# Roestlab/diffusion-deconvolution-dia-msms-data

Hardware: AMD Instinct MI355X
Metric: MS2 windows/s (train step: zero_grad + train_step + backward + clip 10 + AdamW) (higher is better)
Workload: dtype f32; 1 GPU; BASELINE configs[1]: default UNet1d (dim 4, mults 1,2,2,3,3,4,4; 128,847 params), synthetic MS2+MS1 windows 400 RT x 64 m/z, batch 32 per GPU, fp32; global_batch=32, parallelism=dp1

## Files before the change

### diffusion-deconvolution-dia-msms-data_amd/csrc/dq_mfma.h

```cpp
#pragma once
#include <hip/hip_runtime.h>

namespace dq {

typedef float f32x16 __attribute__((ext_vector_type(16)));

__device__ __forceinline__ f32x16 mfma_f32(float a, float b, f32x16 c) { return __builtin_amdgcn_mfma_f32_32x32x2f32(a, b, c, 0, 0, 0); }
__device__ __forceinline__ constexpr int rmap(int r, int half) { return (r & 3) + 8 * (r >> 2) + 4 * half; }
__host__ __device__ __forceinline__ constexpr int la_nj(int C) { return C == 4 ? 2 : (C == 12 ? 6 : (C <= 8 ? 4 : 8)); }
__device__ __forceinline__ constexpr int la_chan(int C, int j, int half) {
  return C == 4 ? 2 * half + j : (C == 12 ? 6 * half + j : rmap(j, half));
}
__host__ __device__ __forceinline__ constexpr int sm_chan(int C, int i, int half) { return C == 12 ? i + 6 * half : (i & 3) + 8 * (i >> 2) + 4 * half; }
__device__ __forceinline__ float swap_half(float v) { return __shfl_xor(v, 32, 64); }

__device__ __forceinline__ f32x16 xty(const f32x16& x, const f32x16& y, f32x16 acc) {
#pragma unroll
  for (int r = 0; r < 16; ++r) acc = mfma_f32(x[r], y[r], acc);
  return acc;
}

__device__ __forceinline__ f32x16 transpose_tile(f32x16 a, float* tile, int col, int half) {
  __builtin_amdgcn_fence(__ATOMIC_ACQ_REL, "wavefront");
  __builtin_amdgcn_wave_barrier();
#pragma unroll
  for (int r = 0; r < 16; ++r) tile[rmap(r, half) * 33 + col] = a[r];
  __builtin_amdgcn_fence(__ATOMIC_ACQ_REL, "wavefront");
  __builtin_amdgcn_wave_barrier();
  f32x16 o;
#pragma unroll
  for (int r = 0; r < 16; ++r) o[r] = tile[col * 33 + rmap(r, half)];
  return o;
}

template <int N>
__device__ __forceinline__ f32x16 mask_same_row(f32x16 a, int col, int half) {
  const int cr = col / N;
#pragma unroll
  for (int r = 0; r < 16; ++r) {
    const int rr = half ? rmap(r, 1) / N : rmap(r, 0) / N;
    a[r] = rr == cr ? a[r] : 0.f;
  }
  return a;
}

}
```

### diffusion-deconvolution-dia-msms-data_amd/csrc/k_attn.hip

```cpp
#include "dq_common.h"
#include "dq_kernels.h"
#include "dq_mfma.h"
#include <cstdlib>

namespace dq {


constexpr float ATT_SCALE = 0.17677669529663687f;
constexpr float LOG2E = 1.4426950408889634f;

__global__ void __launch_bounds__(256) k_rope(float* __restrict__ t0, int64_t bs0, float* __restrict__ t1, int64_t bs1, const float* __restrict__ freqs,
                                              int RT, float sign, int64_t total) {
  float* __restrict__ t = blockIdx.y ? t1 : t0;
  const int64_t batch_stride = blockIdx.y ? bs1 : bs0;
  const int64_t i = blockIdx.x * (int64_t)blockDim.x + threadIdx.x;
  if (i >= total) return;
  const int pos = (int)(i % RT);
  const int pr = (int)((i / RT) % 8);
  const int64_t bh = i / ((int64_t)RT * 8);
  const int64_t b = bh >> 2, h = bh & 3;
  const float ang = (float)pos * freqs[pr];
  float sn, cs;
  sincosf(ang, &sn, &cs);
  sn *= sign;
  float* pa = t + b * batch_stride + (h * 32 + 2 * pr) * RT + pos;
  const float xa = pa[0], xb = pa[RT];
  pa[0] = xa * cs - xb * sn;
  pa[RT] = xb * cs + xa * sn;
}

int launch_rope(float* qk, const float* freqs, int B, int64_t batch_stride, int RT, float sign, hipStream_t s) {
  const int64_t total = (int64_t)B * 4 * 8 * RT;
  if (total == 0) return 0;
  hipLaunchKernelGGL(k_rope, dim3(cdiv(total, 256)), dim3(256), 0, s, qk, batch_stride, (float*)nullptr, (int64_t)0, freqs, RT, sign, total);
  DQ_LAUNCH_CHECK();
  return 0;
}
int launch_rope2(float* q, int64_t q_bs, float* k, int64_t k_bs, const float* freqs, int B, int RT, float sign, hipStream_t s) {
  const int64_t total = (int64_t)B * 4 * 8 * RT;
  if (total == 0) return 0;
  hipLaunchKernelGGL(k_rope, dim3(cdiv(total, 256), 2), dim3(256), 0, s, q, q_bs, k, k_bs, freqs, RT, sign, total);
  DQ_LAUNCH_CHECK();
  return 0;
}

template <bool FAST = true>
__device__ __forceinline__ f32x16 tile_ch_rows(const float* __restrict__ src, int RT, int p0, int col, int half, float mul) {
  f32x16 t;
  if (FAST && p0 + 32 <= RT) {
    const unsigned voff = (unsigned)(p0 + col + 4 * half * RT) * 4u;
#pragma unroll
    for (int r = 0; r < 16; ++r) {
      const float v = *reinterpret_cast<const float*>(reinterpret_cast<const char*>(src + (size_t)((r & 3) + 8 * (r >> 2)) * RT) + voff);
      t[r] = mul == 1.f ? v : v * mul;
    }
    return t;
  }
  const int p = p0 + col;
  const bool ok = p < RT;
  const float* s0 = src + (ok ? p : RT - 1);
  const float m = ok ? mul : 0.f;
#pragma unroll
  for (int r = 0; r < 16; ++r) t[r] = s0[(int64_t)rmap(r, half) * RT] * m;
  return t;
}
__device__ __forceinline__ f32x16 tile_pos_rows(const float* __restrict__ src, int RT, int p0, int col, int half, float mul) {
  f32x16 t;
  const float* row = src + (int64_t)col * RT;
  if ((RT & 3) == 0 && p0 + 32 <= RT) {
#pragma unroll
    for (int q4 = 0; q4 < 4; ++q4) {
      const float4 v = *reinterpret_cast<const float4*>(row + p0 + 8 * q4 + 4 * half);
      if (mul == 1.f) { t[4 * q4 + 0] = v.x; t[4 * q4 + 1] = v.y; t[4 * q4 + 2] = v.z; t[4 * q4 + 3] = v.w; }
      else { t[4 * q4 + 0] = v.x * mul; t[4 * q4 + 1] = v.y * mul; t[4 * q4 + 2] = v.z * mul; t[4 * q4 + 3] = v.w * mul; }
    }
  } else {
#pragma unroll
    for (int r = 0; r < 16; ++r) {
      const int p = p0 + rmap(r, half);
      t[r] = row[p < RT ? p : RT - 1] * (p < RT ? mul : 0.f);
    }
  }
  return t;
}
__device__ __forceinline__ f32x16 rows_scalar(const float* __restrict__ v, int RT, int p0, int half, float fill) {
  f32x16 t;
#pragma unroll
  for (int r = 0; r < 16; ++r) {
    const int p = p0 + rmap(r, half);
    const float x = v[p < RT ? p : RT - 1];
    t[r] = p < RT ? x : fill;
  }
  return t;
}

__global__ void __launch_bounds__(64) k_attn_fwd(const float* __restrict__ q, int64_t q_bs, const float* __restrict__ k, int64_t k_bs,
                                                 const float* __restrict__ v, int64_t v_bs, float* __restrict__ o,
                                                 float* __restrict__ lse, int RT) {
  const int lane = threadIdx.x & 63, col = lane & 31, half = lane >> 5;
  const int bh = blockIdx.y, b = bh >> 2, h = bh & 3;
  const int i0 = blockIdx.x * 32, i = i0 + col;
  const float* qb = q + b * q_bs + (int64_t)h * 32 * RT;
  const float* kb = k + b * k_bs + (int64_t)h * 32 * RT;
  const float* vb = v + b * v_bs + (int64_t)h * 32 * RT;
  const f32x16 Qt = tile_ch_rows<false>(qb, RT, i0, col, half, ATT_SCALE);
  f32x16 Oa = {0};
  float m = -INFINITY, l = 0.f;
  const int jlast = (RT - 1) / 32 * 32;
  auto kblk = [&](int j) { return min(j, jlast); };
  f32x16 Kn = tile_ch_rows<false>(kb, RT, kblk(0), col, half, 1.f);
  f32x16 Vn = tile_pos_rows(vb, RT, kblk(0), col, half, 1.f);
  for (int j0 = 0; j0 < RT; j0 += 32) {
    const f32x16 Kt = Kn, Vx = Vn;
    Kn = tile_ch_rows<false>(kb, RT, kblk(j0 + 32), col, half, 1.f);
    Vn = tile_pos_rows(vb, RT, kblk(j0 + 32), col, half, 1.f);
    f32x16 St = xty(Kt, Qt, f32x16{0});
    float mx = -INFINITY;
#pragma unroll
    for (int r = 0; r < 16; ++r) {
      if (j0 + rmap(r, half) >= RT) St[r] = -INFINITY;
      mx = fmaxf(mx, St[r]);
    }
    mx = fmaxf(mx, swap_half(mx));
    const float mn = fmaxf(m, mx);
    const float al = __builtin_amdgcn_exp2f((m - mn) * LOG2E);
    float ls = 0.f;
#pragma unroll
    for (int r = 0; r < 16; ++r) {
      St[r] = __builtin_amdgcn_exp2f((St[r] - mn) * LOG2E);
      ls += St[r];
    }
    ls += swap_half(ls);
    l = fmaf(l, al, ls);
    m = mn;
#pragma unroll
    for (int r = 0; r < 16; ++r) Oa[r] *= al;
    Oa = xty(Vx, St, Oa);
  }
  if (i < RT) {
    const float rl = 1.0f / l;
    float* ob = o + (int64_t)b * 128 * RT + (int64_t)h * 32 * RT;
#pragma unroll
    for (int r = 0; r < 16; ++r) ob[(int64_t)rmap(r, half) * RT + i] = Oa[r] * rl;
    if (lse && half == 0) lse[(int64_t)bh * RT + i] = m + __logf(l);
  }
}

int launch_attn_fwd(const float* q, int64_t q_bs, const float* k, int64_t k_bs, const float* v, int64_t v_bs, float* o, float* lse,
                    int B, int RT, hipStream_t s) {
  if (B == 0 || RT == 0) return 0;
  hipLaunchKernelGGL(k_attn_fwd, dim3(cdiv(RT, 32), B * 4), dim3(64), 0, s, q, q_bs, k, k_bs, v, v_bs, o, lse, RT);
  DQ_LAUNCH_CHECK();
  return 0;
}

__global__ void __launch_bounds__(64) k_attn_bwd_q(const float* __restrict__ q, int64_t q_bs, const float* __restrict__ k,
                                                   int64_t k_bs, const float* __restrict__ v, int64_t v_bs,
                                                   const float* __restrict__ o, const float* __restrict__ d_o,
                                                   const float* __restrict__ lse, float* __restrict__ delta,
                                                   float* __restrict__ dq, int64_t dq_bs, int RT) {
  const int lane = threadIdx.x & 63, col = lane & 31, half = lane >> 5;
  const int bh = blockIdx.y, b = bh >> 2, h = bh & 3;
  const int i0 = blockIdx.x * 32, i = i0 + col;
  const float* qb = q + b * q_bs + (int64_t)h * 32 * RT;
  const float* kb = k + b * k_bs + (int64_t)h * 32 * RT;
  const float* vb = v + b * v_bs + (int64_t)h * 32 * RT;
  const float* ob = o + (int64_t)b * 128 * RT + (int64_t)h * 32 * RT;
  const float* dob = d_o + (int64_t)b * 128 * RT + (int64_t)h * 32 * RT;
  const int jlast = (RT - 1) / 32 * 32;
  auto kblk = [&](int j) { return min(j, jlast); };
  f32x16 Kn = tile_ch_rows(kb, RT, kblk(0), col, half, 1.f);
  f32x16 Vn = tile_ch_rows(vb, RT, kblk(0), col, half, 1.f);
  f32x16 Xn = tile_pos_rows(kb, RT, kblk(0), col, half, 1.f);
  const f32x16 Qt = tile_ch_rows(qb, RT, i0, col, half, ATT_SCALE);
  const f32x16 dOt = tile_ch_rows(dob, RT, i0, col, half, 1.f);
  float dl = 0.f;
  {
    const f32x16 Ot = tile_ch_rows(ob, RT, i0, col, half, 1.f);
#pragma unroll
    for (int r = 0; r < 16; ++r) dl = fmaf(dOt[r], Ot[r], dl);
    dl += swap_half(dl);
  }
  const float ls = i < RT ? lse[(int64_t)bh * RT + i] : INFINITY;
  f32x16 dQa = {0};
  for (int j0 = 0; j0 < RT; j0 += 32) {
    const f32x16 Kt = Kn, Vt = Vn, Kx = Xn;
    Kn = tile_ch_rows(kb, RT, kblk(j0 + 32), col, half, 1.f);
    Vn = tile_ch_rows(vb, RT, kblk(j0 + 32), col, half, 1.f);
    Xn = tile_pos_rows(kb, RT, kblk(j0 + 32), col, half, 1.f);
    f32x16 St = xty(Kt, Qt, f32x16{0});
    const f32x16 dPt = xty(Vt, dOt, f32x16{0});
#pragma unroll
    for (int r = 0; r < 16; ++r) {
      const float p = (j0 + rmap(r, half) < RT) ? __builtin_amdgcn_exp2f((St[r] - ls) * LOG2E) : 0.f;
      St[r] = p * (dPt[r] - dl);
    }
    dQa = xty(Kx, St, dQa);
  }
  if (i < RT) {
    float* dqb = dq + b * dq_bs + (int64_t)h * 32 * RT;
#pragma unroll
    for (int r = 0; r < 16; ++r) dqb[(int64_t)rmap(r, half) * RT + i] = dQa[r] * ATT_SCALE;
    if (half == 0) delta[(int64_t)bh * RT + i] = dl;
  }
}

__global__ void __launch_bounds__(256, 2) k_attn_bwd_kv(const float* __restrict__ q, int64_t q_bs, const float* __restrict__ k,
                                                     int64_t k_bs, const float* __restrict__ v, int64_t v_bs,
                                                     const float* __restrict__ d_o, const float* __restrict__ lse,
                                                     const float* __restrict__ delta, float* __restrict__ dk, int64_t dk_bs,
                                                     float* __restrict__ dv, int64_t dv_bs, int RT) {
  const int lane = threadIdx.x & 63, col = lane & 31, half = lane >> 5;
  const int wv = __builtin_amdgcn_readfirstlane(threadIdx.x >> 6);
  const int bh = blockIdx.y, b = bh >> 2, h = bh & 3;
  const int j0 = blockIdx.x * 32, j = j0 + col;
  const float* qb = q + b * q_bs + (int64_t)h * 32 * RT;
  const float* kb = k + b * k_bs + (int64_t)h * 32 * RT;
  const float* vb = v + b * v_bs + (int64_t)h * 32 * RT;
  const float* dob = d_o + (int64_t)b * 128 * RT + (int64_t)h * 32 * RT;
  const float* lsb = lse + (int64_t)bh * RT;
  const float* dlb = delta + (int64_t)bh * RT;
  const int ilast = (RT - 1) / 32 * 32;
  f32x16 Qn = tile_ch_rows(qb, RT, min(wv * 32, ilast), col, half, ATT_SCALE), dOn = tile_ch_rows(dob, RT, min(wv * 32, ilast), col, half, 1.f);
  const f32x16 Kt = tile_ch_rows(kb, RT, j0, col, half, 1.f);
  const f32x16 Vt = tile_ch_rows(vb, RT, j0, col, half, 1.f);
  f32x16 dKa = {0}, dVa = {0};
  __shared__ float ttiles[4][32 * 33];
  __shared__ float acc_lds[3][2][16][64];
  float* ttile = ttiles[wv];
  for (int i0 = wv * 32; i0 < RT; i0 += 128) {
    const f32x16 Qt = Qn, dOt = dOn;
    const f32x16 lsr = rows_scalar(lsb, RT, i0, half, INFINITY);
    const f32x16 dlr = rows_scalar(dlb, RT, i0, half, 0.f);
    Qn = tile_ch_rows(qb, RT, min(i0 + 128, ilast), col, half, ATT_SCALE);
    dOn = tile_ch_rows(dob, RT, min(i0 + 128, ilast), col, half, 1.f);
    f32x16 S = xty(Qt, Kt, f32x16{0});
#pragma unroll
    for (int r = 0; r < 16; ++r) S[r] = __builtin_amdgcn_exp2f((S[r] - lsr[r]) * LOG2E);
    {
      const f32x16 dOx = transpose_tile(dOt, ttile, col, half);
      dVa = xty(dOx, S, dVa);
    }
    __builtin_amdgcn_sched_barrier(0);
    f32x16 dP = xty(dOt, Vt, f32x16{0});
#pragma unroll
    for (int r = 0; r < 16; ++r) dP[r] = S[r] * (dP[r] - dlr[r]);
    {
      const f32x16 Qx = transpose_tile(Qt, ttile, col, half);
      dKa = xty(Qx, dP, dKa);
    }
  }
  if (wv > 0) {
#pragma unroll
    for (int r = 0; r < 16; ++r) { acc_lds[wv - 1][0][r][lane] = dKa[r]; acc_lds[wv - 1][1][r][lane] = dVa[r]; }
  }
  __syncthreads();
  if (wv == 0 && j < RT) {
    float* dkb = dk + b * dk_bs + (int64_t)h * 32 * RT;
    float* dvb = dv + b * dv_bs + (int64_t)h * 32 * RT;
#pragma unroll
    for (int r = 0; r < 16; ++r) {
      const float sk = ((dKa[r] + acc_lds[0][0][r][lane]) + acc_lds[1][0][r][lane]) + acc_lds[2][0][r][lane];
      const float sv = ((dVa[r] + acc_lds[0][1][r][lane]) + acc_lds[1][1][r][lane]) + acc_lds[2][1][r][lane];
      dkb[(int64_t)rmap(r, half) * RT + j] = sk;
      dvb[(int64_t)rmap(r, half) * RT + j] = sv;
    }
  }
}

int launch_attn_bwd(const float* q, int64_t q_bs, const float* k, int64_t k_bs, const float* v, int64_t v_bs, const float* o,
                    const float* d_o, const float* lse, float* delta, float* dq, int64_t dq_bs, float* dk, int64_t dk_bs, float* dv,
                    int64_t dv_bs, int B, int RT, hipStream_t s) {
  if (B == 0 || RT == 0) return 0;
  dim3 grid(cdiv(RT, 32), B * 4);
  hipLaunchKernelGGL(k_attn_bwd_q, grid, dim3(64), 0, s, q, q_bs, k, k_bs, v, v_bs, o, d_o, lse, delta, dq, dq_bs, RT);
  DQ_LAUNCH_CHECK();
  hipLaunchKernelGGL(k_attn_bwd_kv, grid, dim3(256), 0, s, q, q_bs, k, k_bs, v, v_bs, d_o, lse, delta, dk, dk_bs, dv, dv_bs, RT);
  DQ_LAUNCH_CHECK();
  return 0;
}

}
```

### diffusion-deconvolution-dia-msms-data_amd/csrc/k_linattn.hip

```cpp
#include "dq_common.h"
#include "dq_kernels.h"
#include "dq_mfma.h"
#include "dq_probe.h"
#include <algorithm>
#include <cstdlib>
#include <string>

namespace dq {

typedef float f32x4 __attribute__((ext_vector_type(4)));
__device__ __forceinline__ f32x16 mfma32(float a, float b, f32x16 c) { return __builtin_amdgcn_mfma_f32_32x32x2f32(a, b, c, 0, 0, 0); }
__device__ __forceinline__ f32x4 mfma4f(float a, float b, f32x4 c) { return __builtin_amdgcn_mfma_f32_4x4x1f32(a, b, c, 0, 0, 0); }
__device__ __forceinline__ constexpr int rowmap(int r, int half) { return (r & 3) + 8 * (r >> 2) + 4 * half; }
__device__ __forceinline__ float swap32(float v) { return swap_half(v); }
__device__ __forceinline__ void wave_fence() {
  __builtin_amdgcn_fence(__ATOMIC_ACQ_REL, "wavefront");
  __builtin_amdgcn_wave_barrier();
}

typedef __bf16 bf16x8 __attribute__((ext_vector_type(8)));
typedef unsigned int u32x4 __attribute__((ext_vector_type(4)));
__host__ __device__ __forceinline__ constexpr int la_nu(int C) { return (3 * (C / 2) + 3) / 4; }
__device__ __forceinline__ bf16x8 as_bf16x8(u32x4 v) { union { u32x4 u; bf16x8 b; } c; c.u = v; return c.b; }
__device__ __forceinline__ void la_split_x(float v, unsigned& d0, unsigned& d1, unsigned& d2) {
  const unsigned vb = __float_as_uint(v);
  const float r = v - __uint_as_float(vb & 0xffff0000u);
  const unsigned rb = __float_as_uint(r);
  const float l = r - __uint_as_float(rb & 0xffff0000u);
  d0 = __builtin_amdgcn_perm(vb, vb, 0x07060706u);
  d1 = __builtin_amdgcn_perm(rb, rb, 0x07060706u);
  d2 = __builtin_amdgcn_perm(__float_as_uint(l), vb, 0x07060302u);
}
__device__ __forceinline__ unsigned la_bf16_image_dword(const float* __restrict__ w_qkv, int C, int o, int half, int u, int e) {
  const int dw = 4 * u + e, j = dw / 3, t = dw % 3;
  if (j >= C / 2) return 0u;
  const float w = w_qkv[o * C + la_chan(C, j, half)] * 1.4426950408889634f;
  const unsigned hb = __float_as_uint(w) & 0xffff0000u;
  const float r = w - __uint_as_float(hb);
  const unsigned mb = __float_as_uint(r) & 0xffff0000u;
  const unsigned lb = __float_as_uint(r - __uint_as_float(mb));
  return t < 2 ? ((hb >> 16) | mb) : ((lb >> 16) | hb);
}

template <int C, int N, bool BF>
__global__ void __launch_bounds__(256) k_linattn_fwd(LinAttn a) {
  static_assert(!BF || (C <= 8 && N > 1), "the bf16 operand image of 12 / 16 channels does not fit the static LDS next to the other images");
  constexpr int NU = la_nu(C);
  constexpr int NB = N >= 32 ? N / 32 : 1;
  constexpr int RW = N >= 32 ? 1 : 32 / N;
  constexpr int NJ = la_nj(C);
  constexpr int SEG = N >= 32 ? 16 : (N >= 8 ? N / 2 : N);
  constexpr bool PARTNER = N >= 8;
  constexpr int CG = C / 4;
  constexpr int NP = NB * 32;
  constexpr bool SEGM = N == 8 || N == 16;
  static_assert(NB <= 2, "rows longer than 64 take the two-pass path (k_la_long.hip)");
  static_assert(C % 4 == 0, "channel count must be a multiple of 4");

  __shared__ __attribute__((aligned(16))) float w2_lds[4 * C * C];
  __shared__ __attribute__((aligned(16))) float xs_lds[4][C * NP];
  constexpr int MS_ROW = C * 32 + 8;
  __shared__ __attribute__((aligned(16))) float ms_lds[4][(SEGM ? RW : 1) * MS_ROW];
  constexpr bool QUAD = N > 1 && N < 32 && !SEGM;
  __shared__ float tiles[QUAD ? 4 : 1][QUAD ? 32 * 33 : 1];
  float* tile = tiles[QUAD ? (threadIdx.x >> 6) : 0];
  DQ_PSTAMP(300000 + C * 100 + N, 0);
#ifdef DQ_KPROBE
  if ((threadIdx.x & 63) == 0 && threadIdx.x > 0 && dq_kprobe_want == 300000 + C * 100 + N)
    dq_kprobe_buf[((blockIdx.y * gridDim.x + blockIdx.x) & 4095) * 16 + 5 + (threadIdx.x >> 6)] = clock64();
#endif
  const int lane = threadIdx.x & 63, col = lane & 31, half = lane >> 5, wv = threadIdx.x >> 6;
  const int rl = N >= 32 ? 0 : col / N;
  const int unit0 = blockIdx.x * 4 + wv, ustride = gridDim.x * 4;
  float Xn[NB][NJ], gpre_r[NJ], gout_r[NJ], bout_r[NJ];
  auto request_unit = [&](int unit) __attribute__((always_inline)) {
    const int rq = unit * RW + rl;
    const int rc = rq < a.rows ? rq : a.rows - 1;
#pragma unroll
    for (int blk = 0; blk < NB; ++blk) {
      const int pos = N >= 32 ? blk * 32 + col : col % N;
#pragma unroll
      for (int j = 0; j < NJ; ++j) {
        const int c = la_chan(C, j, half);
        Xn[blk][j] = a.x[((int64_t)rc * C + (c < C ? c : 0)) * N + pos];
      }
    }
  };
  auto request_x = [&]() __attribute__((always_inline)) {
    request_unit(unit0);
#pragma unroll
    for (int j = 0; j < NJ; ++j) {
      const int c = la_chan(C, j, half);
      gpre_r[j] = a.g_pre[c < C ? c : 0];
      gout_r[j] = a.g_out[c < C ? c : 0];
      bout_r[j] = a.b_out[c < C ? c : 0];
    }
  };
  float bflag = 0.f;
  constexpr int WQ = BF ? 2 * 4 * NU * 64 * 4 : 2 * 4 * NJ * 2 * 32;
  __shared__ __attribute__((aligned(16))) float wqk_lds[N > 1 ? (WQ + 1023) / 1024 * 1024 : 4];
  if (a.prep) {
    constexpr int NQ = N > 1 ? (WQ / 4 + 255) / 256 : 0;
    const float4 v2 = reinterpret_cast<const float4*>(a.prep)[threadIdx.x];
    float4 vq[NQ > 0 ? NQ : 1];
#pragma unroll
    for (int u = 0; u < NQ; ++u) vq[u] = reinterpret_cast<const float4*>(a.prep + (BF ? LA_PREP_BF16 : 1024))[u * 256 + (int)threadIdx.x];
    bflag = a.prep[LA_PREP_BOUNDED];
    request_x();
    DQ_PSTAMP(300000 + C * 100 + N, 9);
    static_assert(sizeof(ms_lds) >= 64 * sizeof(float4), "the dump area of the W2 copy aliases ms_lds");
    float4* w2dst = (int)threadIdx.x < C * C ? reinterpret_cast<float4*>(w2_lds) + threadIdx.x
                                              : reinterpret_cast<float4*>(&ms_lds[0][0]) + (threadIdx.x & 63);
    *w2dst = v2;
#pragma unroll
    for (int u = 0; u < NQ; ++u) reinterpret_cast<float4*>(wqk_lds)[u * 256 + (int)threadIdx.x] = vq[u];
    DQ_PSTAMP(300000 + C * 100 + N, 10);
  } else {
    request_x();
    for (int i = threadIdx.x; i < 4 * C * C; i += blockDim.x) {
      const int c = i % C, cp = (i / C) % C, hd = i / (C * C);
      float s = 0.f;
#pragma unroll
      for (int e = 0; e < 32; ++e) s = fmaf(a.w_out[cp * 128 + hd * 32 + e], a.w_qkv[(256 + hd * 32 + e) * C + c], s);
      w2_lds[i] = s;
    }
  }
  if (N > 1) {
    if (!a.prep && BF) {
      for (int i = threadIdx.x; i < WQ; i += blockDim.x) {
        const int e = i & 3, ln = (i >> 2) & 63, u = (i >> 8) % NU, mh = i / (256 * NU);
        wqk_lds[i] = __uint_as_float(la_bf16_image_dword(a.w_qkv, C, mh * 32 + (ln & 31), ln >> 5, u, e));
      }
    } else if (!a.prep) {
      for (int i = threadIdx.x; i < WQ; i += blockDim.x) {
        const int cc = i & 31, hh = (i >> 5) & 1, j = (i >> 6) % NJ, hd = (i / (64 * NJ)) & 3, m = i / (256 * NJ);
        const int c = la_chan(C, j, hh);
        wqk_lds[i] = c < C ? a.w_qkv[(m * 128 + hd * 32 + cc) * C + c] * 1.4426950408889634f : 0.f;
      }
    }
  }
  float* bnd_lds = &ms_lds[0][0];
  static_assert(sizeof(ms_lds) >= 256 * sizeof(float), "bnd_lds aliases ms_lds");
  float bnd0 = 0.f;
  if (N > 1 && !a.prep) {
    float n2 = 0.f;
    for (int c = 0; c < C; ++c) { const float w = a.w_qkv[threadIdx.x * C + c]; n2 = fmaf(w, w, n2); }
    bnd_lds[threadIdx.x] = n2;
    __syncthreads();
    for (int st = 128; st > 0; st >>= 1) {
      if ((int)threadIdx.x < st) bnd_lds[threadIdx.x] = fmaxf(bnd_lds[threadIdx.x], bnd_lds[threadIdx.x + st]);
      __syncthreads();
    }
    bnd0 = bnd_lds[0];
  }
  if (a.prep) lds_barrier();
  else __syncthreads();
  DQ_PSTAMP(300000 + C * 100 + N, 1);

  float* xs = xs_lds[wv];
  float* ms = ms_lds[wv];
  const float sqC = sqrtf((float)C);
  const float scale = 0.17677669529663687f;
  bool bounded;
  if (a.prep) {
    bounded = __builtin_amdgcn_readfirstlane(__float_as_int(bflag)) != 0;
  } else if (N > 1) {
    float gm = 0.f;
    for (int c = 0; c < C; ++c) gm = fmaxf(gm, fabsf(a.g_pre[c]));
    bounded = 1.4426950408889634f * sqrtf(bnd0) * sqC * gm <= 64.f;
  } else {
    bounded = false;
  }
#pragma unroll
  for (int j = 0; j < NJ; ++j) {
    const bool ok = la_chan(C, j, half) < C;
    gpre_r[j] = ok ? gpre_r[j] : 0.f;
    gout_r[j] = ok ? gout_r[j] : 0.f;
    bout_r[j] = ok ? bout_r[j] : 0.f;
  }
#pragma unroll 1
  for (int unit = unit0; unit * RW < a.rows; unit += ustride) {
  const int row = unit * RW + rl;
  const bool row_ok = row < a.rows;
  float X[NB][NJ], Xh[NB][NJ];
#pragma unroll
  for (int j = 0; j < NJ; ++j) {
    const bool ok = la_chan(C, j, half) < C;
#pragma unroll
    for (int blk = 0; blk < NB; ++blk) X[blk][j] = (row_ok && ok) ? Xn[blk][j] : 0.f;
  }
  if ((unit + ustride) * RW < a.rows) request_unit(unit + ustride);
  wave_fence();
#pragma unroll
  for (int blk = 0; blk < NB; ++blk) {
    float ssq = 0.f;
#pragma unroll
    for (int j = 0; j < NJ; ++j) ssq = fmaf(X[blk][j], X[blk][j], ssq);
    ssq += swap32(ssq);
    const float inv = rms_inv(ssq, sqC);
#pragma unroll
    for (int j = 0; j < NJ; ++j) {
      const int c = la_chan(C, j, half);
      Xh[blk][j] = X[blk][j] * inv * gpre_r[j];
      if (c < C) xs[c * NP + blk * 32 + col] = Xh[blk][j];
    }
  }
  wave_fence();
  u32x4 xp[NB][BF ? NU : 1];
  if (BF) {
#pragma unroll
    for (int blk = 0; blk < NB; ++blk) {
      unsigned dw[4 * NU];
#pragma unroll
      for (int i = 0; i < 4 * NU; ++i) dw[i] = 0u;
#pragma unroll
      for (int j = 0; j < NJ; ++j) la_split_x(Xh[blk][j], dw[3 * j], dw[3 * j + 1], dw[3 * j + 2]);
#pragma unroll
      for (int u = 0; u < NU; ++u) xp[blk][u] = u32x4{dw[4 * u], dw[4 * u + 1], dw[4 * u + 2], dw[4 * u + 3]};
    }
  }

  DQ_PSTAMP(300000 + C * 100 + N, 2);
  float yown[NB][NJ];
#pragma unroll
  for (int blk = 0; blk < NB; ++blk)
#pragma unroll
    for (int j = 0; j < NJ; ++j) yown[blk][j] = 0.f;

  auto add_w2 = [&](int hd, int blk, const float (&p)[C], float f) {
#pragma unroll
    for (int j = 0; j < NJ; ++j) {
      const int cp = la_chan(C, j, half);
      if (cp < C) {
        const float* w = w2_lds + (hd * C + cp) * C;
        float s = 0.f;
#pragma unroll
        for (int c4 = 0; c4 < CG; ++c4) {
          const float4 w4 = *reinterpret_cast<const float4*>(w + 4 * c4);
          s = fmaf(w4.x, p[4 * c4 + 0], fmaf(w4.y, p[4 * c4 + 1], fmaf(w4.z, p[4 * c4 + 2], fmaf(w4.w, p[4 * c4 + 3], s))));
        }
        yown[blk][j] = fmaf(f, s, yown[blk][j]);
      }
    }
  };
  auto chain4 = [&](const float* src, int pitch, int off, int g, const f32x16& t) {
    const float* ar = src + (g * 4 + (lane & 3)) * pitch + off + 4 * half;
    f32x4 t0 = {0.f, 0.f, 0.f, 0.f}, t1 = {0.f, 0.f, 0.f, 0.f};
#pragma unroll
    for (int q4 = 0; q4 < 4; ++q4) {
      const float4 a4 = *reinterpret_cast<const float4*>(ar + 8 * q4);
      t0 = mfma4f(a4.x, t[q4 * 4 + 0], t0); t1 = mfma4f(a4.y, t[q4 * 4 + 1], t1);
      t0 = mfma4f(a4.z, t[q4 * 4 + 2], t0); t1 = mfma4f(a4.w, t[q4 * 4 + 3], t1);
    }
    return t0 + t1;
  };

#pragma unroll 1
  for (int hd = 0; hd < 4; ++hd) {
    if (N == 1) {
      float xf[C];
#pragma unroll
      for (int c = 0; c < C; ++c) xf[c] = xs[c * NP + col];
      add_w2(hd, 0, xf, scale);
      continue;
    }
    float wq[BF ? 1 : NJ], wk[BF ? 1 : NJ];
    u32x4 wkb[BF ? NU : 1];
    if (BF) {
#pragma unroll
      for (int u = 0; u < NU; ++u)
        wkb[u] = reinterpret_cast<const u32x4*>(wqk_lds)[((1 * 4 + hd) * NU + u) * 64 + lane];
    } else {
#pragma unroll
      for (int j = 0; j < NJ; ++j) {
        wq[j] = wqk_lds[(((0 * 4 + hd) * NJ + j) * 2 + half) * 32 + col];
        wk[j] = wqk_lds[(((1 * 4 + hd) * NJ + j) * 2 + half) * 32 + col];
      }
    }
    f32x16 kT[NB];
#pragma unroll
    for (int blk = 0; blk < NB; ++blk) {
      f32x16 ak = {0};
      if (BF) {
#pragma unroll
        for (int u = 0; u < NU; ++u) ak = __builtin_amdgcn_mfma_f32_32x32x16_bf16(as_bf16x8(xp[blk][u]), as_bf16x8(wkb[u]), ak, 0, 0, 0);
      } else {
#pragma unroll
        for (int j = 0; j < NJ; ++j) ak = mfma32(Xh[blk][j], wk[j], ak);
      }
      kT[blk] = ak;
    }
    float krs = 1.f;
    float krs_seg[16 / SEG];
#pragma unroll
    for (int s = 0; s < 16 / SEG; ++s) krs_seg[s] = 1.f;
#pragma unroll
    for (int s0 = 0; s0 < 16; s0 += SEG) {
      float ssum = 0.f;
      if (bounded) {
#pragma unroll
        for (int blk = 0; blk < NB; ++blk)
#pragma unroll
          for (int r = s0; r < s0 + SEG; ++r) {
            const float e = __builtin_amdgcn_exp2f(kT[blk][r]);
            kT[blk][r] = e;
            ssum += e;
          }
      } else {
        float m = -INFINITY;
#pragma unroll
        for (int blk = 0; blk < NB; ++blk)
#pragma unroll
          for (int r = s0; r < s0 + SEG; ++r) m = fmaxf(m, kT[blk][r]);
        if (PARTNER) m = fmaxf(m, swap32(m));
#pragma unroll
        for (int blk = 0; blk < NB; ++blk)
#pragma unroll
          for (int r = s0; r < s0 + SEG; ++r) {
            const float e = __builtin_amdgcn_exp2f(kT[blk][r] - m);
            kT[blk][r] = e;
            ssum += e;
          }
      }
      if (PARTNER) ssum += swap32(ssum);
      const float rs = fast_rcp(ssum);
      if (N >= 32) krs = rs;
      else if (SEGM) krs_seg[s0 / SEG] = rs;
      else {
#pragma unroll
        for (int r = s0; r < s0 + SEG; ++r) kT[0][r] *= rs;
      }
    }
    auto make_q = [&](int blk, float& qs) {
      f32x16 q = {0};
      if (BF) {
#pragma unroll
        for (int u = 0; u < NU; ++u) {
          const u32x4 wqb = reinterpret_cast<const u32x4*>(wqk_lds)[((0 * 4 + hd) * NU + u) * 64 + lane];
          q = __builtin_amdgcn_mfma_f32_32x32x16_bf16(as_bf16x8(wqb), as_bf16x8(xp[blk][u]), q, 0, 0, 0);
        }
      } else {
#pragma unroll
        for (int j = 0; j < NJ; ++j) q = mfma32(wq[j], Xh[blk][j], q);
      }
      float ssum = 0.f;
      if (bounded) {
#pragma unroll
        for (int r = 0; r < 16; ++r) {
          q[r] = __builtin_amdgcn_exp2f(q[r]);
          ssum += q[r];
        }
      } else {
        float m = q[0];
#pragma unroll
        for (int r = 1; r < 16; ++r) m = fmaxf(m, q[r]);
        m = fmaxf(m, swap32(m));
#pragma unroll
        for (int r = 0; r < 16; ++r) {
          q[r] = __builtin_amdgcn_exp2f(q[r] - m);
          ssum += q[r];
        }
      }
      ssum += swap32(ssum);
      qs = scale * fast_rcp(ssum);
      return q;
    };

    if (N >= 32) {
      wave_fence();
#pragma unroll
      for (int g = 0; g < CG; ++g) {
        f32x4 mt = {0.f, 0.f, 0.f, 0.f};
#pragma unroll
        for (int blk = 0; blk < NB; ++blk) mt += chain4(xs, NP, blk * 32, g, kT[blk]);
#pragma unroll
        for (int i = 0; i < 4; ++i) {
          const float v = (mt[i] + swap32(mt[i])) * krs;
          if (half == 0) ms[(g * 4 + i) * 32 + col] = v;
        }
      }
      wave_fence();
#pragma unroll
      for (int blk = 0; blk < NB; ++blk) {
        float qs;
        const f32x16 q = make_q(blk, qs);
        float P[C];
#pragma unroll
        for (int g = 0; g < CG; ++g) {
          const f32x4 pp = chain4(ms, 32, 0, g, q);
#pragma unroll
          for (int i = 0; i < 4; ++i) P[g * 4 + i] = pp[i] + swap32(pp[i]);
        }
        add_w2(hd, blk, P, qs);
      }
    } else if (SEGM) {
      wave_fence();
#pragma unroll
      for (int s = 0; s < 16 / SEG; ++s)
#pragma unroll
        for (int g = 0; g < CG; ++g) {
          const float* ar = xs + (g * 4 + (lane & 3)) * NP + 4 * half;
          f32x4 t0 = {0.f, 0.f, 0.f, 0.f}, t1 = {0.f, 0.f, 0.f, 0.f};
#pragma unroll
          for (int q4 = s * SEG / 4; q4 < (s + 1) * SEG / 4; ++q4) {
            const float4 a4 = *reinterpret_cast<const float4*>(ar + 8 * q4);
            t0 = mfma4f(a4.x, kT[0][q4 * 4 + 0], t0); t1 = mfma4f(a4.y, kT[0][q4 * 4 + 1], t1);
            t0 = mfma4f(a4.z, kT[0][q4 * 4 + 2], t0); t1 = mfma4f(a4.w, kT[0][q4 * 4 + 3], t1);
          }
          const f32x4 mt = t0 + t1;
#pragma unroll
          for (int i = 0; i < 4; ++i) {
            const float v = (mt[i] + swap32(mt[i])) * krs_seg[s];
            if (half == 0) ms[s * MS_ROW + (g * 4 + i) * 32 + col] = v;
          }
        }
      wave_fence();
      float qs;
      const f32x16 q = make_q(0, qs);
      float P[C];
#pragma unroll
      for (int g = 0; g < CG; ++g) {
        const f32x4 pp = chain4(ms + rl * MS_ROW, 32, 0, g, q);
#pragma unroll
        for (int i = 0; i < 4; ++i) P[g * 4 + i] = pp[i] + swap32(pp[i]);
      }
      add_w2(hd, 0, P, qs);
    } else {
      float qs;
      const f32x16 q = make_q(0, qs);
      const f32x16 Kd = transpose_tile(kT[0], tile, col, half);
      f32x16 st = {0};
      st = xty(Kd, q, st);
      st = mask_same_row<N>(st, col, half);
      float R[C];
#pragma unroll
      for (int g = 0; g < CG; ++g) {
        const f32x4 rr = chain4(xs, NP, 0, g, st);
#pragma unroll
        for (int i = 0; i < 4; ++i) R[g * 4 + i] = rr[i] + swap32(rr[i]);
      }
      add_w2(hd, 0, R, qs);
    }
  }
  DQ_PSTAMP(300000 + C * 100 + N, 3);


#pragma unroll
  for (int blk = 0; blk < NB; ++blk) {
    const int pos = N >= 32 ? blk * 32 + col : col % N;
    float yv[NJ];
    float ssq = 0.f;
#pragma unroll
    for (int j = 0; j < NJ; ++j) {
      const int c = la_chan(C, j, half);
      yv[j] = c < C ? yown[blk][j] + bout_r[j] : 0.f;
      ssq = fmaf(yv[j], yv[j], ssq);
    }
    ssq += swap32(ssq);
    const float inv = rms_inv(ssq, sqC);
#pragma unroll
    for (int j = 0; j < NJ; ++j) {
      const int c = la_chan(C, j, half);
      if (row_ok && c < C) {
        const int64_t off = ((int64_t)row * C + c) * N + pos;
        if (a.ypre) a.ypre[off] = yv[j];
        a.y[off] = fmaf(yv[j] * gout_r[j], inv, X[blk][j]);
      }
    }
  }
  }
  DQ_PSTAMP(300000 + C * 100 + N, 4);
}

static int la_num_cus() {
  static const int v = [] { int d = 0; hipDeviceProp_t pr; return (hipGetDevice(&d) == hipSuccess && hipGetDeviceProperties(&pr, d) == hipSuccess) ? pr.multiProcessorCount : 256; }();
  return v;
}
template <int C>
static int linattn_fwd_n(const LinAttn& a, hipStream_t s) {
#define DQ_LA(NN)                                                                      \
  case NN: {                                                                           \
    constexpr int RW = NN >= 32 ? 1 : 32 / NN;                                         \
     \
    constexpr bool CAN_BF = C <= 8 && NN > 1 && !(C == 8 && NN <= 8);                  \
    const int units = cdiv(a.rows, RW);                                                \
    const int grid = cdiv(units, 4);   \
    hipLaunchKernelGGL((k_linattn_fwd<C, NN, CAN_BF>), dim3(grid), dim3(256), 0, s, a); \
    break;                                                                             \
  }
  switch (a.n) {
    DQ_LA(1) DQ_LA(2) DQ_LA(4) DQ_LA(8) DQ_LA(16) DQ_LA(32) DQ_LA(64)
    default:
      set_error("linattn_fwd: m/z length " + std::to_string(a.n) + " is not built (powers of two up to 64)");
      return 2;
  }
#undef DQ_LA
  DQ_LAUNCH_CHECK();
  return 0;
}

struct LaPrepMulti { LaPrepItem it[LA_PREP_MAX]; PrepCopy cp[PREP_COPY_MAX]; int count; };
__global__ void __launch_bounds__(256) k_linattn_prepare(LaPrepMulti m) {
  if ((int)blockIdx.x >= m.count) {
    const PrepCopy& c = m.cp[blockIdx.x - m.count];
    for (int base = 0; base < c.n; base += 8 * 256) {
      float v[8];
#pragma unroll
      for (int u = 0; u < 8; ++u) { const int i = base + u * 256 + (int)threadIdx.x; v[u] = c.src[i < c.n ? i : 0]; }
#pragma unroll
      for (int u = 0; u < 8; ++u) { const int i = base + u * 256 + (int)threadIdx.x; if (i < c.n) c.dst[i] = v[u]; }
    }
    return;
  }
  const LaPrepItem& it = m.it[blockIdx.x];
  const int C = it.C, NJ = la_nj(C);
  {
    float sv[4];
#pragma unroll
    for (int u = 0; u < 4; ++u) {
      const int i = u * 256 + (int)threadIdx.x;
      const int ic = i < 4 * C * C ? i : 0;
      const int c = ic % C, cp = (ic / C) % C, hd = ic / (C * C);
      float s = 0.f;
#pragma unroll
      for (int e = 0; e < 32; ++e) s = fmaf(it.w_out[cp * 128 + hd * 32 + e], it.w_qkv[(256 + hd * 32 + e) * C + c], s);
      sv[u] = s;
    }
#pragma unroll
    for (int u = 0; u < 4; ++u) { const int i = u * 256 + (int)threadIdx.x; if (i < 4 * C * C) it.prep[i] = sv[u]; }
  }
  const int WQ = 2 * 4 * NJ * 2 * 32;
  {
    float v[16];
#pragma unroll
    for (int u = 0; u < 16; ++u) {
      const int i = u * 256 + (int)threadIdx.x;
      const int cc = i & 31, hh = (i >> 5) & 1, j = (i >> 6) % NJ, hd = (i / (64 * NJ)) & 3, mm = (i / (256 * NJ)) & 1;
      const int c = la_chan(C, j, hh);
      v[u] = 0.f;
      if (u * 256 < WQ) v[u] = it.w_qkv[(mm * 128 + hd * 32 + cc) * C + (c < C ? c : 0)];
    }
#pragma unroll
    for (int u = 0; u < 16; ++u) {
      const int i = u * 256 + (int)threadIdx.x;
      const int hh = (i >> 5) & 1, j = (i >> 6) % NJ;
      const int c = la_chan(C, j, hh);
      if (i < WQ) it.prep[1024 + i] = c < C ? v[u] * 1.4426950408889634f : 0.f;
    }
  }
  if (C <= 8) {
    const int NU = la_nu(C);
#pragma unroll 1
    for (int u = 0; u < NU; ++u) {
      const int e = (int)threadIdx.x & 3, ln = (int)threadIdx.x >> 2, dw = 4 * u + e, j = dw / 3, t = dw % 3;
      const bool live = j < C / 2;
      const int c = live ? la_chan(C, j, ln >> 5) : 0;
      float w[8];
#pragma unroll
      for (int mh = 0; mh < 8; ++mh) w[mh] = it.w_qkv[(mh * 32 + (ln & 31)) * C + c];
#pragma unroll
      for (int mh = 0; mh < 8; ++mh) {
        const float ws = w[mh] * 1.4426950408889634f;
        const unsigned hb = __float_as_uint(ws) & 0xffff0000u;
        const float r = ws - __uint_as_float(hb);
        const unsigned mb = __float_as_uint(r) & 0xffff0000u;
        const unsigned lb = __float_as_uint(r - __uint_as_float(mb));
        const unsigned v = !live ? 0u : (t < 2 ? ((hb >> 16) | mb) : ((lb >> 16) | hb));
        it.prep[LA_PREP_BF16 + (mh * NU + u) * 256 + (int)threadIdx.x] = __uint_as_float(v);
      }
    }
  }
  __shared__ float red[256];
  {
    float n2 = 0.f;
    for (int c = 0; c < C; ++c) { const float w = it.w_qkv[threadIdx.x * C + c]; n2 = fmaf(w, w, n2); }
    red[threadIdx.x] = n2;
    __syncthreads();
    for (int st = 128; st > 0; st >>= 1) {
      if ((int)threadIdx.x < st) red[threadIdx.x] = fmaxf(red[threadIdx.x], red[threadIdx.x + st]);
      __syncthreads();
    }
    if (threadIdx.x == 0) {
      float gm = 0.f;
      for (int c = 0; c < C; ++c) gm = fmaxf(gm, fabsf(it.g_pre[c]));
      const float bound = 1.4426950408889634f * sqrtf(red[0]) * sqrtf((float)C) * gm;
      it.prep[LA_PREP_BOUNDED] = (bound <= 64.f) ? 1.f : 0.f;
    }
  }
  if (C >= 8) {
    const int S = C / 2;
    for (int i = threadIdx.x; i < 12 * S * 64; i += 256) {
      const int l = i & 63, st = (i >> 6) % S, g = i / (64 * S);
      const int mrow = l & 31, c = sm_chan(C, st, l >> 5);
      float v = 0.f;
      if (g < 8) v = c < C ? it.w_qkv[((g >> 2) * 128 + (g & 3) * 32 + mrow) * C + c] * 1.4426950408889634f : 0.f;
      else v = (mrow < C && c < C) ? it.prep[((g - 8) * C + mrow) * C + c] : 0.f;
      it.prep[LA_PREP_SMALL + i] = v;
    }
    const int CPL = C / 4;
    constexpr int NR = 4 * 64 * LA_ROWS_LANE_FLOATS / 256;
    float rv[NR];
#pragma unroll
    for (int u = 0; u < NR; ++u) {
      const int i = u * 256 + (int)threadIdx.x;
      const int k = i % LA_ROWS_LANE_FLOATS, l = (i / LA_ROWS_LANE_FLOATS) & 63, hd = i / (64 * LA_ROWS_LANE_FLOATS);
      const int g = l >> 4, ii = l & 15;
      const int ci = (ii & 3) < CPL ? CPL * (ii >> 2) + (ii & 3) : -1;
      const float* src = it.w_qkv;
      int off = 0;
      bool ok = false;
      float mul = 1.f;
      if (k < 16) {
        const int m = k >> 3, e = k & 7, t = e / CPL, s = e % CPL;
        ok = e < 2 * CPL;
        off = (m * 128 + hd * 32 + 16 * (ok ? t : 0) + ii) * C + CPL * g + s;
        mul = 1.4426950408889634f;
      } else if (k < 20) {
        const int s = k - 16;
        ok = s < CPL && ci >= 0;
        src = it.prep;
        off = ok ? (hd * C + CPL * g + s) * C + ci : 0;
      } else {
        const int e = k - 20, m = e >> 3, t = (e >> 2) & 1, r = e & 3;
        ok = ci >= 0;
        off = (m * 128 + hd * 32 + 16 * t + 4 * g + r) * C + (ok ? ci : 0);
      }
      const float v = src[off];
      rv[u] = ok ? v * mul : 0.f;
    }
#pragma unroll
    for (int u = 0; u < NR; ++u) it.prep[LA_PREP_ROWS + u * 256 + (int)threadIdx.x] = rv[u];
  }
}
int launch_linattn_prepare(const LaPrepItem* items, int count, hipStream_t s, const PrepCopy* copies, int n_copies) {
  if (count + n_copies == 0) return 0;
  DQ_REQUIRE(count <= LA_PREP_MAX && n_copies <= PREP_COPY_MAX, "linattn prepare: too many layers / copies");
  LaPrepMulti m;
  m.count = count;
  for (int i = 0; i < n_copies; ++i) m.cp[i] = copies[i];
  for (int i = 0; i < count; ++i) {
    DQ_REQUIRE(items[i].C % 4 == 0 && items[i].C <= 16, "linattn prepare: unsupported channel count");
    m.it[i] = items[i];
  }
  hipLaunchKernelGGL(k_linattn_prepare, dim3(count + n_copies), dim3(256), 0, s, m);
  DQ_LAUNCH_CHECK();
  return 0;
}

LaFwdForm la_fwd_form(const LinAttn& a) {
  if (!la_short_row(a.n)) return LA_FWD_LONG;
  if (a.prep && la_small_usable(a.C, a.n) && a.rows >= la_small_min_rows() &&
      (((uintptr_t)a.prep | (uintptr_t)a.x | (uintptr_t)a.y | (uintptr_t)a.ypre) & 15) == 0)
    return LA_FWD_SMALL;
  if (a.prep && la_rows_fwd_usable(a.C, a.n) && a.rows >= la_rows_bwd_min_rows() && (((uintptr_t)a.x | (uintptr_t)a.prep) & 15) == 0)
    return LA_FWD_ROWS;
  return LA_FWD_REG;
}

int launch_linattn_fwd(const LinAttn& a, hipStream_t s) {
  DQ_REQUIRE(a.x && a.y && a.w_qkv && a.w_out && a.b_out && a.g_pre && a.g_out, "linattn_fwd: missing operand");
  if (a.rows == 0) return 0;
  switch (la_fwd_form(a)) {
    case LA_FWD_LONG: return launch_linattn_fwd_long(a, s);
    case LA_FWD_SMALL: return launch_la_small_fwd(a, s);
    case LA_FWD_ROWS: return launch_la_rows_fwd(a, s);
    case LA_FWD_REG: break;
  }
  switch (a.C) {
    case 4: return linattn_fwd_n<4>(a, s);
    case 8: return linattn_fwd_n<8>(a, s);
    case 12: return linattn_fwd_n<12>(a, s);
    case 16: return linattn_fwd_n<16>(a, s);
    default: set_error("linattn_fwd: unsupported channel count " + std::to_string(a.C)); return 2;
  }
}

}
```

Measured before the change: 10300 windows/s.

## Emulate fp32 attention matmuls with split-bf16 MFMA (six-product) accumulation

Replaces the fp32 32x32x2 MFMA chains in the attention forward, dQ and dK/dV kernels with a three-way bf16 split (high/mid/low) and six bf16 32x32x16 MFMA products per tile. The goal is higher matrix throughput while keeping accuracy close to fp32. The dK/dV kernel is also restructured: both Q and dO tiles are transposed into separate LDS buffers up front, and S and dP are computed before the two accumulation matmuls. The cost is extra VALU work to split every tile each iteration and more LDS. Dropping some low-order cross terms may slightly change numerics.

```diff
diff --git a/diffusion-deconvolution-dia-msms-data_amd/csrc/dq_mfma.h b/diffusion-deconvolution-dia-msms-data_amd/csrc/dq_mfma.h
--- a/diffusion-deconvolution-dia-msms-data_amd/csrc/dq_mfma.h
+++ b/diffusion-deconvolution-dia-msms-data_amd/csrc/dq_mfma.h
@@ -20,17 +20,23 @@
   return acc;
 }
 
-__device__ __forceinline__ f32x16 transpose_tile(f32x16 a, float* tile, int col, int half) {
+__device__ __forceinline__ void transpose_put(const f32x16& a, float* tile, int col, int half) {
   __builtin_amdgcn_fence(__ATOMIC_ACQ_REL, "wavefront");
   __builtin_amdgcn_wave_barrier();
 #pragma unroll
   for (int r = 0; r < 16; ++r) tile[rmap(r, half) * 33 + col] = a[r];
+}
+__device__ __forceinline__ f32x16 transpose_get(const float* tile, int col, int half) {
   __builtin_amdgcn_fence(__ATOMIC_ACQ_REL, "wavefront");
   __builtin_amdgcn_wave_barrier();
   f32x16 o;
 #pragma unroll
   for (int r = 0; r < 16; ++r) o[r] = tile[col * 33 + rmap(r, half)];
   return o;
+}
+__device__ __forceinline__ f32x16 transpose_tile(f32x16 a, float* tile, int col, int half) {
+  transpose_put(a, tile, col, half);
+  return transpose_get(tile, col, half);
 }
 
 template <int N>
@@ -44,4 +50,46 @@
   return a;
 }
 
+typedef __bf16 bf16x8 __attribute__((ext_vector_type(8)));
+typedef unsigned int u32x4 __attribute__((ext_vector_type(4)));
+__device__ __forceinline__ bf16x8 as_bf16x8(u32x4 v) { union { u32x4 u; bf16x8 b; } c; c.u = v; return c.b; }
+__device__ __forceinline__ f32x16 mfma_bf16(u32x4 a, u32x4 b, f32x16 c) { return __builtin_amdgcn_mfma_f32_32x32x16_bf16(as_bf16x8(a), as_bf16x8(b), c, 0, 0, 0); }
+
+struct Split16 { u32x4 h[2], m[2], l[2]; };
+typedef float f32x2 __attribute__((ext_vector_type(2)));
+typedef __bf16 bf16x2 __attribute__((ext_vector_type(2)));
+__device__ __forceinline__ Split16 split_tile(const f32x16& x) {
+  Split16 t;
+#pragma unroll
+  for (int s = 0; s < 2; ++s)
+#pragma unroll
+    for (int p = 0; p < 4; ++p) {
+      const f32x2 v = {x[8 * s + 2 * p], x[8 * s + 2 * p + 1]};
+      const bf16x2 h = __builtin_convertvector(v, bf16x2);
+      const f32x2 r = v - __builtin_convertvector(h, f32x2);
+      const bf16x2 m = __builtin_convertvector(r, bf16x2);
+      const bf16x2 l = __builtin_convertvector(r - __builtin_convertvector(m, f32x2), bf16x2);
+      t.h[s][p] = __builtin_bit_cast(unsigned, h);
+      t.m[s][p] = __builtin_bit_cast(unsigned, m);
+      t.l[s][p] = __builtin_bit_cast(unsigned, l);
+    }
+  return t;
 }
+template <bool MIRROR = false>
+__device__ __forceinline__ f32x16 xty6(const Split16& x, const Split16& y, f32x16 acc) {
+#pragma unroll
+  for (int s = 0; s < 2; ++s) acc = MIRROR ? mfma_bf16(x.h[s], y.l[s], acc) : mfma_bf16(x.l[s], y.h[s], acc);
+#pragma unroll
+  for (int s = 0; s < 2; ++s) acc = MIRROR ? mfma_bf16(x.l[s], y.h[s], acc) : mfma_bf16(x.h[s], y.l[s], acc);
+#pragma unroll
+  for (int s = 0; s < 2; ++s) acc = mfma_bf16(x.m[s], y.m[s], acc);
+#pragma unroll
+  for (int s = 0; s < 2; ++s) acc = MIRROR ? mfma_bf16(x.h[s], y.m[s], acc) : mfma_bf16(x.m[s], y.h[s], acc);
+#pragma unroll
+  for (int s = 0; s < 2; ++s) acc = MIRROR ? mfma_bf16(x.m[s], y.h[s], acc) : mfma_bf16(x.h[s], y.m[s], acc);
+#pragma unroll
+  for (int s = 0; s < 2; ++s) acc = mfma_bf16(x.h[s], y.h[s], acc);
+  return acc;
+}
+
+}
diff --git a/diffusion-deconvolution-dia-msms-data_amd/csrc/k_attn.hip b/diffusion-deconvolution-dia-msms-data_amd/csrc/k_attn.hip
--- a/diffusion-deconvolution-dia-msms-data_amd/csrc/k_attn.hip
+++ b/diffusion-deconvolution-dia-msms-data_amd/csrc/k_attn.hip
@@ -103,7 +103,7 @@
   const float* qb = q + b * q_bs + (int64_t)h * 32 * RT;
   const float* kb = k + b * k_bs + (int64_t)h * 32 * RT;
   const float* vb = v + b * v_bs + (int64_t)h * 32 * RT;
-  const f32x16 Qt = tile_ch_rows<false>(qb, RT, i0, col, half, ATT_SCALE);
+  const Split16 Qs = split_tile(tile_ch_rows<false>(qb, RT, i0, col, half, ATT_SCALE));
   f32x16 Oa = {0};
   float m = -INFINITY, l = 0.f;
   const int jlast = (RT - 1) / 32 * 32;
@@ -114,7 +114,7 @@
     const f32x16 Kt = Kn, Vx = Vn;
     Kn = tile_ch_rows<false>(kb, RT, kblk(j0 + 32), col, half, 1.f);
     Vn = tile_pos_rows(vb, RT, kblk(j0 + 32), col, half, 1.f);
-    f32x16 St = xty(Kt, Qt, f32x16{0});
+    f32x16 St = xty6(split_tile(Kt), Qs, f32x16{0});
     float mx = -INFINITY;
 #pragma unroll
     for (int r = 0; r < 16; ++r) {
@@ -135,7 +135,7 @@
     m = mn;
 #pragma unroll
     for (int r = 0; r < 16; ++r) Oa[r] *= al;
-    Oa = xty(Vx, St, Oa);
+    Oa = xty6(split_tile(Vx), split_tile(St), Oa);
   }
   if (i < RT) {
     const float rl = 1.0f / l;
@@ -172,8 +172,9 @@
   f32x16 Kn = tile_ch_rows(kb, RT, kblk(0), col, half, 1.f);
   f32x16 Vn = tile_ch_rows(vb, RT, kblk(0), col, half, 1.f);
   f32x16 Xn = tile_pos_rows(kb, RT, kblk(0), col, half, 1.f);
-  const f32x16 Qt = tile_ch_rows(qb, RT, i0, col, half, ATT_SCALE);
+  const Split16 Qs = split_tile(tile_ch_rows(qb, RT, i0, col, half, ATT_SCALE));
   const f32x16 dOt = tile_ch_rows(dob, RT, i0, col, half, 1.f);
+  const Split16 dOs = split_tile(dOt);
   float dl = 0.f;
   {
     const f32x16 Ot = tile_ch_rows(ob, RT, i0, col, half, 1.f);
@@ -188,14 +189,14 @@
     Kn = tile_ch_rows(kb, RT, kblk(j0 + 32), col, half, 1.f);
     Vn = tile_ch_rows(vb, RT, kblk(j0 + 32), col, half, 1.f);
     Xn = tile_pos_rows(kb, RT, kblk(j0 + 32), col, half, 1.f);
-    f32x16 St = xty(Kt, Qt, f32x16{0});
-    const f32x16 dPt = xty(Vt, dOt, f32x16{0});
+    f32x16 St = xty6(split_tile(Kt), Qs, f32x16{0});
+    const f32x16 dPt = xty6(split_tile(Vt), dOs, f32x16{0});
 #pragma unroll
     for (int r = 0; r < 16; ++r) {
       const float p = (j0 + rmap(r, half) < RT) ? __builtin_amdgcn_exp2f((St[r] - ls) * LOG2E) : 0.f;
       St[r] = p * (dPt[r] - dl);
     }
-    dQa = xty(Kx, St, dQa);
+    dQa = xty6(split_tile(Kx), split_tile(St), dQa);
   }
   if (i < RT) {
     float* dqb = dq + b * dq_bs + (int64_t)h * 32 * RT;
@@ -222,33 +223,38 @@
   const float* dlb = delta + (int64_t)bh * RT;
   const int ilast = (RT - 1) / 32 * 32;
   f32x16 Qn = tile_ch_rows(qb, RT, min(wv * 32, ilast), col, half, ATT_SCALE), dOn = tile_ch_rows(dob, RT, min(wv * 32, ilast), col, half, 1.f);
-  const f32x16 Kt = tile_ch_rows(kb, RT, j0, col, half, 1.f);
-  const f32x16 Vt = tile_ch_rows(vb, RT, j0, col, half, 1.f);
+  const Split16 Ks = split_tile(tile_ch_rows(kb, RT, j0, col, half, 1.f));
+  const Split16 Vs = split_tile(tile_ch_rows(vb, RT, j0, col, half, 1.f));
   f32x16 dKa = {0}, dVa = {0};
-  __shared__ float ttiles[4][32 * 33];
+  __shared__ float ttiles[4][2][32 * 33];
   __shared__ float acc_lds[3][2][16][64];
-  float* ttile = ttiles[wv];
+  float* tq = ttiles[wv][0];
+  float* tdo = ttiles[wv][1];
   for (int i0 = wv * 32; i0 < RT; i0 += 128) {
-    const f32x16 Qt = Qn, dOt = dOn;
     const f32x16 lsr = rows_scalar(lsb, RT, i0, half, INFINITY);
     const f32x16 dlr = rows_scalar(dlb, RT, i0, half, 0.f);
-    Qn = tile_ch_rows(qb, RT, min(i0 + 128, ilast), col, half, ATT_SCALE);
-    dOn = tile_ch_rows(dob, RT, min(i0 + 128, ilast), col, half, 1.f);
-    f32x16 S = xty(Qt, Kt, f32x16{0});
-#pragma unroll
-    for (int r = 0; r < 16; ++r) S[r] = __builtin_amdgcn_exp2f((S[r] - lsr[r]) * LOG2E);
+    f32x16 S, dP;
     {
-      const f32x16 dOx = transpose_tile(dOt, ttile, col, half);
-      dVa = xty(dOx, S, dVa);
+      const f32x16 Qt = Qn;
+      Qn = tile_ch_rows(qb, RT, min(i0 + 128, ilast), col, half, ATT_SCALE);
+      transpose_put(Qt, tq, col, half);
+      S = xty6<true>(split_tile(Qt), Ks, f32x16{0});
+    }
+    {
+      const f32x16 dOt = dOn;
+      dOn = tile_ch_rows(dob, RT, min(i0 + 128, ilast), col, half, 1.f);
+      transpose_put(dOt, tdo, col, half);
+      dP = xty6<true>(split_tile(dOt), Vs, f32x16{0});
+    }
+#pragma unroll
+    for (int r = 0; r < 16; ++r) {
+      S[r] = __builtin_amdgcn_exp2f((S[r] - lsr[r]) * LOG2E);
+      dP[r] = S[r] * (dP[r] - dlr[r]);
     }
     __builtin_amdgcn_sched_barrier(0);
-    f32x16 dP = xty(dOt, Vt, f32x16{0});
-#pragma unroll
-    for (int r = 0; r < 16; ++r) dP[r] = S[r] * (dP[r] - dlr[r]);
-    {
-      const f32x16 Qx = transpose_tile(Qt, ttile, col, half);
-      dKa = xty(Qx, dP, dKa);
-    }
+    dVa = xty6(split_tile(transpose_get(tdo, col, half)), split_tile(S), dVa);
+    __builtin_amdgcn_sched_barrier(0);
+    dKa = xty6(split_tile(transpose_get(tq, col, half)), split_tile(dP), dKa);
   }
   if (wv > 0) {
 #pragma unroll
diff --git a/diffusion-deconvolution-dia-msms-data_amd/csrc/k_linattn.hip b/diffusion-deconvolution-dia-msms-data_amd/csrc/k_linattn.hip
--- a/diffusion-deconvolution-dia-msms-data_amd/csrc/k_linattn.hip
+++ b/diffusion-deconvolution-dia-msms-data_amd/csrc/k_linattn.hip
@@ -18,10 +18,7 @@
   __builtin_amdgcn_wave_barrier();
 }
 
-typedef __bf16 bf16x8 __attribute__((ext_vector_type(8)));
-typedef unsigned int u32x4 __attribute__((ext_vector_type(4)));
 __host__ __device__ __forceinline__ constexpr int la_nu(int C) { return (3 * (C / 2) + 3) / 4; }
-__device__ __forceinline__ bf16x8 as_bf16x8(u32x4 v) { union { u32x4 u; bf16x8 b; } c; c.u = v; return c.b; }
 __device__ __forceinline__ void la_split_x(float v, unsigned& d0, unsigned& d1, unsigned& d2) {
   const unsigned vb = __float_as_uint(v);
   const float r = v - __uint_as_float(vb & 0xffff0000u);
```

Measured after the change: 10420 windows/s (median of 6 runs). 1.01x the previous value.
